# heathsc/bs_call

Hardware: AMD Instinct MI355X
Metric: genome positions called/sec (higher is better)
Workload: dtype f64; 1 GPU; configs[1]: synthetic chr22-sized contig, 50000000 positions at 30x WGBS (L-pileup generator), pile-ups resident in HBM, one contig per GPU; positions_per_gpu=50000000, coverage=30

## Files before the change

bs_call_amd/_lib.py:

```python
import ctypes as C
import os

HERE = os.path.dirname(os.path.abspath(__file__))
LIB_PATH = os.environ.get("BSCALL_AMD_LIB") or os.path.join(HERE, "lib", "libbscall_amd.so")

EXPORTS = (
    "bsc_abi_version",
    "bsc_last_error",
    "bsc_params_default",
    "bsc_create",
    "bsc_destroy",
    "bsc_get_tables",
    "bsc_phred_table",
    "bsc_call_sites",
    "bsc_alloc_host",
    "bsc_free_host",
    "bsc_call_sites_device",
    "bsc_accumulate",
    "bsc_accumulate_device",
    "bsc_block_status",
    "bsc_last_accumulate_ms",
    "bsc_call_block",
    "bsc_block_submit",
    "bsc_block_fetch",
    "bsc_block_submit_to",
    "bsc_synth_reads_host",
    "bsc_vcf_records",
# ... 412 lines not shown
    vp, u64, u32, i32 = C.c_void_p, C.c_uint64, C.c_uint32, C.c_int
    L.bsc_abi_version.restype = i32
    L.bsc_abi_version.argtypes = []
    if L.bsc_abi_version() != ABI_VERSION:
        raise ImportError("%s has ABI %d, this package mirrors ABI %d: rebuild with `make`" % (LIB_PATH, L.bsc_abi_version(), ABI_VERSION))
    L.bsc_last_error.restype = C.c_char_p
    L.bsc_last_error.argtypes = []
    L.bsc_params_default.restype = None
    L.bsc_params_default.argtypes = [C.POINTER(Params)]
    L.bsc_create.restype = i32
    L.bsc_create.argtypes = [C.POINTER(Params), C.POINTER(vp)]
    L.bsc_destroy.restype = i32
    L.bsc_destroy.argtypes = [vp]
    L.bsc_get_tables.restype = i32
    L.bsc_get_tables.argtypes = [vp, vp, vp]
    L.bsc_phred_table.restype = i32
    L.bsc_phred_table.argtypes = [vp, vp]
    L.bsc_call_sites.restype = i32
    L.bsc_call_sites.argtypes = [vp, vp, vp, u64, vp, u32, vp]
    L.bsc_alloc_host.restype = vp
    L.bsc_alloc_host.argtypes = [u64]
    L.bsc_free_host.restype = None
    L.bsc_free_host.argtypes = [vp]
    L.bsc_call_sites_device.restype = i32
    L.bsc_call_sites_device.argtypes = [vp, vp, vp, u64, vp, u32, vp, vp]
    L.bsc_accumulate.restype = i32
    L.bsc_accumulate.argtypes = [vp, vp, u32, vp, u64, u32, u32, vp]
    L.bsc_accumulate_device.restype = i32
    L.bsc_accumulate_device.argtypes = [vp, vp, u32, vp, u64, u32, u32, vp, vp]
    L.bsc_block_status.restype = i32
# ... 452 lines not shown
```

bs_call_amd/caller.py:

```python
import ctypes as C

import numpy as np

from . import _lib
from .abi import GT_METH, PILEUP, SITE_STATS, TEMPLATE, VCF_CORE, VCF_REC

SYNTH_NRUNS = 1


class BscError(RuntimeError):
    def __init__(self, code, msg):
        super().__init__("bscall_amd error %d: %s" % (code, msg))
        self.code = code


class BscInexactWarning(UserWarning):
    """Some pile-up sums left the range where the reference's float sums are exact (BSC_WARN_INEXACT)."""


def _check(rc):
    if rc == 1:
        import warnings

        warnings.warn(_lib.load().bsc_last_error().decode("utf-8", "replace"), BscInexactWarning, stacklevel=3)
# ... 252 lines not shown
        at = 0
        for k in pieces:
            z.write(data[at : at + k])
            at += k
            parts.append(z.take())
        if at < len(data):
            z.write(data[at:])
        parts.append(z.close())
        return b"".join(parts)

    def tables(self):
        q = np.zeros((44, 5), dtype=np.float64)
        lf = np.zeros(256, dtype=np.float64)
        _check(self._L.bsc_get_tables(self._h, _ptr(q), _ptr(lf)))
        return q, lf

    def call_sites(self, pile, ref, out_stride=200, out=None, skip=None):
        pile = np.ascontiguousarray(pile, dtype=PILEUP)
        ref = np.ascontiguousarray(ref, dtype=np.uint8)
        n = len(pile)
        if len(ref) != n:
            raise ValueError("pile and ref differ in length")
        if out is None:
            out = np.zeros(n, dtype=GT_METH) if out_stride == 200 else np.zeros((n, out_stride), dtype=np.uint8)
        if skip is None:
            skip = np.zeros(n, dtype=np.uint8)
        _check_dest("out", out, n * out_stride)
        _check_dest("skip", skip, n)
        _check(self._L.bsc_call_sites(self._h, _ptr(pile), _ptr(ref), n, _ptr(out), out_stride, _ptr(skip)))
        return out, skip
# ... 1104 lines not shown
```

bs_call_amd/csrc/bscall_api.c:

```c
#ifndef __HIP_PLATFORM_AMD__
#define __HIP_PLATFORM_AMD__ 1
#endif
#include <hip/hip_runtime_api.h>
#include <math.h>
#include <pthread.h>
#include <stdarg.h>
#include <stdio.h>
#include <stdlib.h>
#include <string.h>

#include "../../include/bscall_amd.h"
#include "devtables.h"
#include "bsmath.h"
#include "bsmath_tables.h"
#include "synth.h"
#include "dbsnpdev_core.h"
#include "tabix_int.h"

int bsc_dev_launch_call(const void *cts, const void *ref, uint64_t n, void *out, uint32_t out_dw, void *skip,
                        const void *tb, void *het_list, void *counters, int num_cus, void *stream, void *ev_start,
                        void *ev_mid, void *ev_stop);
int bsc_dev_launch_accumulate(const void *rd, const void *bin_off, const void *seq, uint32_t x, uint32_t y, uint32_t min_qual, void *cts,
                              void *counters, int num_cus, void *stream);
int bsc_dev_launch_bin_reads(const void *tpl, uint32_t nr, const void *seq, uint64_t seq_bytes, uint32_t x, uint32_t y, void *tflag,
                             void *bin_cnt, void *bin_off, void *bin_cur, void *scan_tmp, size_t scan_tmp_bytes, void *rd,
                             void *counters, void *stream);
uint32_t bsc_dev_n_bins(uint32_t n_sites);
int bsc_dev_launch_site_stats(const void *core, const void *gtm, uint32_t gtm_stride, const void *dbsnp, uint32_t n,
                              const void *tb, const void *logp, const void *carry_in, void *carry_out, void *stats,
                              void *pairs, int num_cus, void *stream);
int bsc_dev_launch_gc_cov_gtm(const void *core, const void *gtm, uint32_t gtm_stride, uint32_t n, const void *gc_bins, uint32_t n_bins,
                              uint32_t start_pos, void *table, int num_cus, void *stream);
int bsc_dev_launch_meth_eval(void *pairs, const void *tb, const void *logp, void *stats, const void *ovf_list,
                             const void *counters, int num_cus, void *stream);
int bsc_dev_scan_tmp_bytes(uint32_t n, size_t *bytes);
int bsc_dev_launch_stream_probe(const void *cts, const void *ref, uint64_t n, void *out, void *skip, int num_cus,
// ... 287 lines not shown
  size_t cap_fscr;
  hipEvent_t ev_rchain[2];
  int ev_rchain_valid;
  hipEvent_t ev_raw[2];
  int ev_raw_valid;
  int ref_resident;
  hipEvent_t ev_acc[2];
  int ev_acc_valid;
  hipStream_t s_in, s_out;
  hipEvent_t ev_in[2], ev_k[2], ev_out[2];
  void *p_cts[2], *p_ref[2], *p_out[2], *p_skip[2];
  size_t p_cap_cts[2], p_cap_ref[2], p_cap_out[2], p_cap_skip[2];
  int pipe_ready;
  int profiling;
#define BSC_EV_RING 32
  hipEvent_t ev[BSC_EV_RING][3];
  uint64_t ev_count;
};

static __thread char bsc_errbuf[512];

static int bsc_fail(int code, const char *fmt, ...) {
  va_list ap;
  va_start(ap, fmt);
  vsnprintf(bsc_errbuf, sizeof bsc_errbuf, fmt, ap);
  va_end(ap);
  return code;
}

typedef struct {
  int prev;
// ... 98 lines not shown
    ctx->q_prob[q][3] = t->ln_k_half[q] = log(0.5 + k);
    ctx->q_prob[q][4] = t->ln_k_one[q] = log(1.0 + k);
  }
  t->lfact[0] = t->lfact[1] = 0.0;
  double l = 0.0;
  for (int i = 2; i < 256; i++) {
    l += log((double)i);
    t->lfact[i] = l;
  }
  memcpy(t->log_tab, bsm_log_tab, sizeof t->log_tab);
  memcpy(t->exp_tab, bsm_exp_tab, sizeof t->exp_tab);
  t->under_conv = ctx->params.under_conv;
  t->over_conv = ctx->params.over_conv;
  t->lrb = log(ctx->params.ref_bias);
  t->lrb1 = log(0.5 * (1.0 + ctx->params.ref_bias));
}

int bsc_create(const bsc_params *params, bsc_context **out) {
  if (!out) return bsc_fail(BSC_ERR_ARG, "bsc_create: out is NULL");
  *out = NULL;
  bsc_params p;
  if (params) p = *params;
  else bsc_params_default(&p);
  if (!(p.under_conv >= 0.0 && p.under_conv < 1.0) || !(p.over_conv >= 0.0 && p.over_conv < 1.0) || !(p.ref_bias > 0.0))
    return bsc_fail(BSC_ERR_ARG, "bsc_create: conversion rates must be in [0,1) and ref_bias > 0");
  if (!((1.0 - p.under_conv) - p.over_conv >= 0x1p-20))
    return bsc_fail(BSC_ERR_ARG, "bsc_create: under_conv + over_conv must be < 1 (by at least 2^-20)");
  if (p.min_qual < 1) p.min_qual = 1;
  if (p.min_qual > 43) p.min_qual = 43;

// ... 235 lines not shown
  hipFree(ctx->d_raw);
  hipFree(ctx->d_rseq);
  hipFree(ctx->d_rms);
  hipFree(ctx->d_pprof);
  hipFree(ctx->d_pmax);
  hipFree(ctx->d_pused);
  hipFree(ctx->d_pmask);
  if (ctx->h_prep) hipHostFree(ctx->h_prep);
  hipFree(ctx->d_carry);
  hipFree(ctx->d_logp);
  hipFree(ctx->d_vout);
  hipFree(ctx->d_vdb);
  if (ctx->h_stage) hipHostFree(ctx->h_stage);
  if (ctx->h_cnt) hipHostFree(ctx->h_cnt);
  for (int r = 0; r < BSC_EV_RING; r++)
    for (int i = 0; i < 3; i++)
      if (ctx->ev[r][i]) hipEventDestroy(ctx->ev[r][i]);
  free(ctx);
  return BSC_OK;
}

int bsc_get_tables(const bsc_context *ctx, double *q_prob_44x5, double *lfact_256) {
  if (!ctx) return bsc_fail(BSC_ERR_ARG, "bsc_get_tables: ctx is NULL");
  if (q_prob_44x5) memcpy(q_prob_44x5, ctx->q_prob, sizeof ctx->q_prob);
  if (lfact_256) memcpy(lfact_256, ctx->host_tables.lfact, sizeof ctx->host_tables.lfact);
  return BSC_OK;
}

static int bsc_reserve(void **p, size_t *cap, size_t need) {
  if (need <= *cap) return BSC_OK;
  if (*p) {
    hipError_t e = hipFree(*p);
    *p = NULL;
// ... 37 lines not shown
int bsc_call_sites_device(bsc_context *ctx, const void *d_cts, const void *d_ref, uint64_t n, void *d_out,
                          uint32_t out_stride, void *d_skip, void *stream) {
  if (!ctx) return bsc_fail(BSC_ERR_ARG, "bsc_call_sites_device: ctx is NULL");
  int rc = bsc_check_stride(out_stride);
  if (rc) return rc;
  if (n == 0) return BSC_OK;
  if (!d_cts || !d_ref || !d_out || !d_skip) return bsc_fail(BSC_ERR_ARG, "bsc_call_sites_device: NULL buffer");
  if (((uintptr_t)d_cts & 15u) || ((uintptr_t)d_out & 15u))
    return bsc_fail(BSC_ERR_ARG, "bsc_call_sites_device: d_cts and d_out must be 16-byte aligned");
  BSC_ENTER(ctx);
  hipStream_t s = (hipStream_t)stream;
  uint64_t done = 0;
  while (done < n) {
    uint64_t m = n - done;
    if (m > ctx->max_launch) m = ctx->max_launch;
    rc = bsc_reserve(&ctx->d_het, &ctx->cap_het, (size_t)((m + 63u) / 64u) * 8u);
    if (rc) return rc;
    int e = bsc_dev_launch_call((const char *)d_cts + done * 104u, (const char *)d_ref + done, m,
                                (char *)d_out + done * out_stride, out_stride / 4u, (char *)d_skip + done,
                                ctx->d_tables, ctx->d_het, ctx->d_counters, ctx->num_cus, s,
                                ctx->profiling ? ctx->ev[ctx->ev_count % BSC_EV_RING][0] : NULL,
                                ctx->profiling ? ctx->ev[ctx->ev_count % BSC_EV_RING][1] : NULL,
                                ctx->profiling ? ctx->ev[ctx->ev_count % BSC_EV_RING][2] : NULL);
    if (ctx->profiling) ctx->ev_count++;
    if (e) return bsc_fail(BSC_ERR_HIP, "kernel launch failed: %s", hipGetErrorString((hipError_t)e));
    done += m;
  }
  ctx->sites += n;
  return BSC_OK;
}

#define BSC_PIPE_CHUNK (1u << 20)

static int bsc_pipe_init(bsc_context *ctx) {
  if (ctx->pipe_ready) return BSC_OK;
  HIP_TRY(hipStreamCreateWithFlags(&ctx->s_in, hipStreamNonBlocking));
  HIP_TRY(hipStreamCreateWithFlags(&ctx->s_out, hipStreamNonBlocking));
  for (int b = 0; b < 2; b++) {
// ... 553 lines not shown
  ctx->reads_fused = fused != 0;
  return BSC_OK;
}

int bsc_debug_fail_summary_alloc(bsc_context *ctx, int on) {
  if (!ctx) return bsc_fail(BSC_ERR_ARG, "bsc_debug_fail_summary_alloc: ctx is NULL");
  ctx->dbg_fail_summary = on != 0;
  return BSC_OK;
}

int bsc_set_profiling(bsc_context *ctx, int enable) {
  if (!ctx) return bsc_fail(BSC_ERR_ARG, "bsc_set_profiling: ctx is NULL");
  BSC_ENTER(ctx);
  if (enable && !ctx->ev[0][0])
    for (int r = 0; r < BSC_EV_RING; r++)
      for (int i = 0; i < 3; i++) HIP_TRY(hipEventCreate(&ctx->ev[r][i]));
  ctx->profiling = enable != 0;
  ctx->ev_count = 0;
  return BSC_OK;
}

int bsc_kernel_ms_history(bsc_context *ctx, uint32_t age, float *call_ms, float *fisher_ms) {
  if (!ctx) return bsc_fail(BSC_ERR_ARG, "bsc_kernel_ms_history: ctx is NULL");
  if (!ctx->profiling || age >= ctx->ev_count || age >= BSC_EV_RING)
    return bsc_fail(BSC_ERR_ARG, "bsc_kernel_ms_history: no profiled launch %u launches back (the last %d are kept)", age, BSC_EV_RING);
  BSC_ENTER(ctx);
  hipEvent_t *ev = ctx->ev[(ctx->ev_count - 1u - age) % BSC_EV_RING];
  HIP_TRY(hipEventSynchronize(ev[2]));
  float a = 0.f, b = 0.f;
  HIP_TRY(hipEventElapsedTime(&a, ev[0], ev[1]));
  HIP_TRY(hipEventElapsedTime(&b, ev[1], ev[2]));
  if (call_ms) *call_ms = a;
  if (fisher_ms) *fisher_ms = b;
  return BSC_OK;
}

int bsc_last_kernel_ms(bsc_context *ctx, float *call_ms, float *fisher_ms) { return bsc_kernel_ms_history(ctx, 0, call_ms, fisher_ms); }

int bsc_stream_probe_ms(bsc_context *ctx, const void *d_cts, const void *d_ref, uint64_t n, void *d_out, void *d_skip,
                        int reps, void *stream, float *ms) {
  if (!ctx || !d_cts || !d_ref || !d_out || !d_skip || !ms) return bsc_fail(BSC_ERR_ARG, "bsc_stream_probe_ms: NULL argument");
  if (((uintptr_t)d_cts & 15u) || ((uintptr_t)d_out & 15u))
    return bsc_fail(BSC_ERR_ARG, "bsc_stream_probe_ms: d_cts and d_out must be 16-byte aligned");
  BSC_ENTER(ctx);
  hipEvent_t a, b;
  HIP_TRY(hipEventCreate(&a));
  HIP_TRY(hipEventCreate(&b));
  float best = 0.f;
// ... 3738 lines not shown
```

bs_call_amd/csrc/bsmath.h:

```cpp
#ifndef BSCALL_AMD_BSMATH_H
#define BSCALL_AMD_BSMATH_H

#include <stdint.h>

#include "bsmath_tables.h"

#if defined(__HIPCC__)
#define BSM_FN __host__ __device__ static __forceinline__
#else
#define BSM_FN static inline __attribute__((always_inline))
#endif

#define BSM_FMA(a, b, c) __builtin_fma((a), (b), (c))

BSM_FN uint64_t bsm_bits(double x) {
  uint64_t u;
  __builtin_memcpy(&u, &x, 8);
  return u;
}
BSM_FN double bsm_from_bits(uint64_t u) {
  double x;
  __builtin_memcpy(&x, &u, 8);
  return x;
}
// ... 104 lines not shown
BSM_FN double bsm_lfact_big_t(int n, const double *logtab) {
  const double x = (double)(n + 1);
  const double t = bsm_log_t(x, logtab);
  const double z = 1.0 / x;
  const double y = z * z;
  double w = y * -1.63092934096575273989e-03;
  w = y * (8.36339918996282139126e-04 + w);
  w = y * (-5.95187557450339963135e-04 + w);
  w = y * (7.93650558643019558500e-04 + w);
  w = y * (-2.77777777728775536470e-03 + w);
  w = z * (8.33333333333329678849e-02 + w);
  w = 4.18938533204672725052e-01 + w;
  return (x - 0.5) * (t - 1.0) + w;
}

#if !defined(__HIPCC__)
BSM_FN double bsm_log(double x) { return bsm_log_t(x, bsm_log_tab); }
BSM_FN double bsm_exp(double x) { return bsm_exp_t(x, bsm_exp_tab); }
BSM_FN double bsm_lfact_big(int n) { return bsm_lfact_big_t(n, bsm_log_tab); }
#endif

#endif
```

bs_call_amd/csrc/callmath.h:

```cpp
#ifndef BSCALL_AMD_CALLMATH_H
#define BSCALL_AMD_CALLMATH_H

#include <hip/hip_runtime.h>
#include <stdint.h>

#include "bsmath.h"

#ifndef BSC_DMA_AUX
#define BSC_DMA_AUX 2
#endif
#define IN_DW 26
#define OUT_DW 50
#define MAX_OUT_DW 52
#define SLOT_DW (64 * IN_DW)

#define WAVE_LDS_ORDER()                                     \
  do {                                                       \
    __builtin_amdgcn_fence(__ATOMIC_RELEASE, "wavefront");   \
    __builtin_amdgcn_wave_barrier();                         \
    __builtin_amdgcn_fence(__ATOMIC_ACQUIRE, "wavefront");   \
  } while (0)

__device__ static __forceinline__ unsigned lane_rank(unsigned long long m) {
  return __builtin_amdgcn_mbcnt_hi((uint32_t)(m >> 32), __builtin_amdgcn_mbcnt_lo((uint32_t)m, 0u));
// ... 170 lines not shown
  const uint64_t db = bsm_bits(d);
  const bool allones = ((uint32_t)db & ((uint32_t)(db >> 32) | 0xfff00000u)) == 0xffffffffu;
  if (__builtin_expect(__any(allones), 0)) {
    s0 = allones ? n0 / d : s0;
    s1 = allones ? n1 / d : s1;
    s2 = allones ? n2 / d : s2;
  }
  s0 = s0 < -1.0 ? -1.0 : (s0 > 1.0 ? 1.0 : s0);
  Z0 = 0.5 * (lmt * s0 + 2.0 - lpt);
  s1 = s1 < -1.0 ? -1.0 : (s1 > 1.0 ? 1.0 : s1);
  Z1 = 0.5 * (lmt * s1 + 2.0 - lpt);
  s2 = s2 < -1.0 ? -1.0 : (s2 > 1.0 ? 1.0 : s2);
  Z2 = 0.5 * (lmt * s2 + 2.0 - lpt);
}

#define PT_Q 44
#define PT_A 0
#define PT_B 1
#define PT_C 2
#define PT_D 3
#define PT_E 4
#define PT_WORDS (5 * PT_Q)
__device__ static __forceinline__ double pure_log_entry(unsigned idx, double l, double t, const double *s_k, const double *logtab) {
  const unsigned id = idx / PT_Q, q = idx - id * PT_Q;
  const double lpt = l + t, lmt = l - t;
  const double Zc = 0.5 * (lmt * -1.0 + 2.0 - lpt), Zd = 0.5 * (lmt * 1.0 + 2.0 - lpt);
  const double k = s_k[q];
  double x;
  switch (id) {
    case PT_A: x = 1.0 - Zc + k; break;
    case PT_B: x = 1.0 - 0.5 * Zc + k; break;
    case PT_C: x = 0.5 * (1.0 - Zc) + k; break;
    case PT_D: x = Zd + k; break;
    default: x = 0.5 * Zd + k; break;
  }
  return bsm_log_t(x, logtab);
}

__device__ static __forceinline__ void dma16(const void *g, void *lds_wave_base) {
  __builtin_amdgcn_global_load_lds((const __attribute__((address_space(1))) void *)g,
                                   (__attribute__((address_space(3))) void *)lds_wave_base, 16, 0, BSC_DMA_AUX);
}

__device__ static __forceinline__ double lfact_dev(int x, const double *lf, const double *logtab) {
  return x < 256 ? lf[x] : bsm_lfact_big_t(x, logtab);
}

__device__ static double fisher_dev(int c0, int c1, int c2, int c3, const double *lf, const double *logtab,
                                    const uint64_t *exptab) {
#define LF(x) lfact_dev((x), lf, logtab)
  const int row0 = c0 + c1, row1 = c2 + c3, col0 = c0 + c2, col1 = c1 + c3;
  const int n = row0 + row1;
// ... 75 lines not shown
```

bs_call_amd/csrc/devtables.h:

```cpp
#ifndef BSCALL_AMD_DEVTABLES_H
#define BSCALL_AMD_DEVTABLES_H

#include <stdint.h>

typedef struct {
  double k[44], ln_k[44], ln_k_half[44], ln_k_one[44];
  double lfact[256];
  double log_tab[256];
  unsigned long long exp_tab[256];
  double under_conv, over_conv;
  double lrb, lrb1;
  double phred_thr[64][4];
  unsigned char phred_base[64];
} bsc_dev_tables;

#define BSC_CNT_HET_LIST 0
#define BSC_CNT_COVERED 1
#define BSC_CNT_SPAN 13
#define BSC_CNT_INEXACT 14
#define BSC_CNT_ERR 15
#define BSC_CNT_RECORDS 16
#define BSC_CNT_OVF 17
#define BSC_CNT_DEEP 18
#define BSC_CNT_WORDS 19

#define BSC_TERR_LEFT 1
#define BSC_TERR_ORI 2
#define BSC_TERR_STRAND 3
// ... 43 lines not shown
```

bs_call_amd/csrc/fused.hip:

```cpp
#include <hip/hip_runtime.h>
#include <stdint.h>
#include <stdlib.h>
#include <string.h>

#include "accdev.h"
#include "bsmath.h"
#include "callmath.h"
#include "devtables.h"
#include "sitestats_dev.h"

#ifndef FW
#define FW 16
#endif
#ifndef BSC_CHAIN_STAGGER
#define BSC_CHAIN_STAGGER 0
#endif
#define FT 60
#define FT2 62
#ifndef BSC_RUN_CAP
#define BSC_RUN_CAP 32
#endif
#define SUM_DW 12
#define F_COV_LDS 256
#define F_WORDS (SS_COV + F_COV_LDS * 6)
// ... 311 lines not shown
    s_lnk[tid] = tb->ln_k[tid];
    s_half[tid] = tb->ln_k_half[tid];
    s_one[tid] = tb->ln_k_one[tid];
  }
  if (tid < 256) {
    s_logtab[tid] = tb->log_tab[tid];
    s_exptab[tid] = tb->exp_tab[tid];
    s_pthr[tid] = (&tb->phred_thr[0][0])[tid];
  }
  if (tid < 64) s_pbase[tid] = tb->phred_base[tid];
  if (tid < 12) s_cnt[tid] = 0;
  if (a.with_stats) {
    for (unsigned i = tid; i < F_WORDS; i += 64 * FW) h[i] = 0;
    for (unsigned i = tid; i < 4 * F_PAIR * F_PAIR; i += 64 * FW) s_pair[i] = 0;
  }
  __syncthreads();
  if (tid < PT_WORDS) s_ptab[tid] = pure_log_entry(tid, K_COLD(l), K_COLD(t), s_k, s_logtab);
  if (tid >= 256 && tid < 306) {
    const unsigned r = (tid - 256u) / 10u, g = (tid - 256u) % 10u;
    int ga, gb;
    f_alleles((int)g, ga, gb);
    s_prior[tid - 256u] = r == 0 ? 0.0 : (ga == (int)r && gb == (int)r ? K_COLD(lrb) : ((ga == (int)r || gb == (int)r) ? K_COLD(lrb1) : 0.0));
  }
  __syncthreads();
  if (BSC_CHAIN_STAGGER)
    for (unsigned i = 0; i < wid; i++) __builtin_amdgcn_s_sleep(BSC_CHAIN_STAGGER);

  uint32_t *slot = lds_slot[wid];
  uint32_t *sg = s_gw[wid];
  uint16_t *srf = s_rf[wid];
  uint16_t *spd = s_pend[wid];
  int64_t ref_lo, ref_hi;
// ... 915 lines not shown
```

bs_call_amd/csrc/kernels.hip:

```cpp
#include <hip/hip_runtime.h>
#include <stdint.h>

#include "bsmath.h"
#include "callmath.h"
#include "devtables.h"
#include "synth.h"

#ifndef TILE
#define TILE 256
#endif
#ifndef BSC_TILES_PER_WAVE
#define BSC_TILES_PER_WAVE 16
#endif
#ifndef BSC_WAVES_PER_SIMD
#define BSC_WAVES_PER_SIMD 4
#endif

template <bool FULL>
__global__ __launch_bounds__(TILE, BSC_WAVES_PER_SIMD) void bsc_call_kernel_t(const uint32_t *__restrict__ cts,
                                                                      const uint8_t *__restrict__ ref,
                                                                      uint64_t n_sites, uint64_t wt_begin,
                                                                      uint64_t wt_end, uint32_t *__restrict__ out,
                                                                      uint32_t out_dw, uint8_t *__restrict__ skip,
                                                                      const bsc_dev_tables *__restrict__ tb,
                                                                      uint32_t *__restrict__ het_list,
                                                                      unsigned long long *__restrict__ counters) {
  __shared__ __attribute__((aligned(16))) uint32_t lds_slot[TILE / 64][SLOT_DW];
  __shared__ double s_k[44], s_lnk[44], s_half[44], s_one[44];
#ifdef BSC_TABLES_GLOBAL
  const double *const s_logtab = tb->log_tab;
  const unsigned long long *const s_exptab = tb->exp_tab;
#else
  __shared__ double s_logtab[256];
  __shared__ unsigned long long s_exptab[256];
#endif
  __shared__ unsigned int s_cnt[12];
  __shared__ double s_ptab[PT_WORDS];
  __shared__ uint8_t s_pairs[TILE / 64][256];

  const unsigned tid = threadIdx.x;
  const unsigned lane = tid & 63u;
  const unsigned wid = __builtin_amdgcn_readfirstlane(tid >> 6);
  if (tid < 44) {
    s_k[tid] = tb->k[tid];
    s_lnk[tid] = tb->ln_k[tid];
    s_half[tid] = tb->ln_k_half[tid];
    s_one[tid] = tb->ln_k_one[tid];
  }
#ifndef BSC_TABLES_GLOBAL
  for (unsigned i = tid; i < 256; i += TILE) {
    s_logtab[i] = tb->log_tab[i];
    s_exptab[i] = tb->exp_tab[i];
  }
#endif
  if (tid < 12) s_cnt[tid] = 0;
  const double l = 1.0 - tb->under_conv;
  const double t = tb->over_conv;
  const double lrb = tb->lrb, lrb1 = tb->lrb1;
  __syncthreads();
  for (unsigned i = tid; i < PT_WORDS; i += TILE) s_ptab[i] = pure_log_entry(i, l, t, s_k, s_logtab);
  __syncthreads();

  uint32_t *slot = lds_slot[wid];
  const uint32_t wave_stride = gridDim.x * (TILE / 64);
  const uint32_t wt_last = (uint32_t)wt_end;
  for (uint32_t wt = (uint32_t)wt_begin + blockIdx.x * (TILE / 64) + wid; wt < wt_last; wt += wave_stride) {
    const uint64_t site0 = (uint64_t)wt * 64;
    const unsigned nvalid = FULL ? 64u : (unsigned)((n_sites - site0) < 64 ? (n_sites - site0) : 64);
    const bool full = FULL;
    const uint64_t site = site0 + lane;
    const bool valid = FULL || lane < nvalid;
    const unsigned rf = valid ? ref[site] : 0u;

    uint32_t w[IN_DW];
    if (full) {
// ... 7 lines not shown
      for (int i = 0; i < IN_DW / 2; i++) {
        const uint2 v = rec[i];
        w[2 * i] = v.x;
        w[2 * i + 1] = v.y;
      }
    } else {
#pragma unroll
      for (int i = 0; i < IN_DW; i++) w[i] = valid ? cts[site * IN_DW + i] : 0u;
    }
#include "call_body.inc"
    const bool het = covered && ((0x16Eu >> mxi) & 1u);
    if (covered) {
      atomicAdd(&s_cnt[0], 1u);
      atomicAdd(&s_cnt[1 + mxi], 1u);
    }
    {
      const unsigned long long m = __ballot(het);
      if (lane == 0) {
        reinterpret_cast<unsigned long long *>(het_list)[wt] = m;
        if (m) atomicAdd(&s_cnt[11], (unsigned)__popcll(m));
      }
    }
    if (valid) skip[site] = covered ? 0 : 1;

#pragma unroll 1
    for (unsigned half = 0; half < 2; half++) {
      __builtin_amdgcn_wave_barrier();
      const bool mine = valid && (lane >> 5) == half;
      auto write_record = [&](auto *rec) {
        if (covered) {
#pragma unroll
          for (int j = 0; j < 8; j++) rec[j] = make_uint2(cnt[j], 0u);
          rec[8] = make_uint2(qpack0 & 0xffu, (qpack0 >> 8) & 0xffu);
          rec[9] = make_uint2((qpack0 >> 16) & 0xffu, qpack0 >> 24);
          rec[10] = make_uint2(qpack1 & 0xffu, (qpack1 >> 8) & 0xffu);
// ... 19 lines not shown
      if (full) {
        __builtin_amdgcn_wave_barrier();
        const unsigned nvec = 32u * out_dw / 4u;
        uint4 *dst = reinterpret_cast<uint4 *>(out + (site0 + half * 32u) * out_dw);
        const uint4 *srcv = reinterpret_cast<const uint4 *>(slot);
#pragma unroll
        for (unsigned v = 0; v < 7; v++) {
          const unsigned idx = v * 64u + lane;
          if (idx < nvec) {
            typedef unsigned int u32x4 __attribute__((ext_vector_type(4)));
            __builtin_nontemporal_store(reinterpret_cast<const u32x4 *>(srcv)[idx], reinterpret_cast<u32x4 *>(dst) + idx);
          }
        }
      }
    }
  }

  __syncthreads();
  if (tid < 12 && s_cnt[tid]) atomicAdd(&counters[BSC_CNT_COVERED + tid], (unsigned long long)s_cnt[tid]);
}

#define FI_THREADS 256
#define FI_LIST 2048
extern "C" __global__ __launch_bounds__(FI_THREADS) void bsc_fisher_kernel(const uint32_t *__restrict__ cts,
                                                                           uint32_t *__restrict__ out, uint32_t out_dw,
                                                                           const bsc_dev_tables *__restrict__ tb,
                                                                           const unsigned long long *__restrict__ masks,
                                                                           uint32_t n_tiles, uint32_t chunk_tiles) {
  __shared__ double s_lf[256];
  __shared__ double s_logtab[256];
  __shared__ unsigned long long s_exptab[256];
  __shared__ uint32_t s_scan[FI_THREADS + 1];
  __shared__ uint32_t s_list[FI_LIST];
  const unsigned tid = threadIdx.x;
  s_lf[tid] = tb->lfact[tid];
  s_logtab[tid] = tb->log_tab[tid];
  s_exptab[tid] = tb->exp_tab[tid];
  const uint32_t per = (chunk_tiles + FI_THREADS - 1) / FI_THREADS;
  for (uint32_t c0 = blockIdx.x * chunk_tiles; c0 < n_tiles; c0 += gridDim.x * chunk_tiles) {
    const uint32_t c1 = min(c0 + chunk_tiles, n_tiles);
    const uint32_t t0 = min(c0 + tid * per, c1), t1 = min(t0 + per, c1);
    uint32_t mine = 0;
    for (uint32_t t = t0; t < t1; t++) mine += (uint32_t)__popcll(masks[t]);
    __syncthreads();
    s_scan[tid + 1] = mine;
    if (tid == 0) s_scan[0] = 0;
    __syncthreads();
    if (tid < 64) {
      uint32_t a = s_scan[4 * tid + 1], b = a + s_scan[4 * tid + 2], c = b + s_scan[4 * tid + 3], d = c + s_scan[4 * tid + 4];
      uint32_t run = d;
#pragma unroll
      for (int off = 1; off < 64; off <<= 1) {
        const uint32_t v = __shfl_up(run, off);
        if ((int)tid >= off) run += v;
      }
      const uint32_t base = run - d;
      s_scan[4 * tid + 1] = base + a;
      s_scan[4 * tid + 2] = base + b;
      s_scan[4 * tid + 3] = base + c;
      s_scan[4 * tid + 4] = base + d;
    }
    __syncthreads();
    const uint32_t total = s_scan[FI_THREADS], first = s_scan[tid];
    for (uint32_t w0 = 0; w0 < total; w0 += FI_LIST) {
      if (w0) __syncthreads();
      if (first < w0 + FI_LIST && first + mine > w0) {
        uint32_t k = first;
        for (uint32_t t = t0; t < t1; t++) {
          unsigned long long m = masks[t];
          while (m) {
            const unsigned bit = (unsigned)__builtin_ctzll(m);
            m &= m - 1ull;
            if (k >= w0 && k < w0 + FI_LIST) s_list[k - w0] = t * 64u + bit;
            k++;
          }
        }
      }
      __syncthreads();
      const uint32_t cnt = min((uint32_t)FI_LIST, total - w0);
      for (uint32_t i = tid; i < cnt; i += FI_THREADS) {
        const uint64_t site = s_list[i];
        const uint32_t *p = cts + site * IN_DW;
        uint32_t f[8], r[8];
#pragma unroll
        for (int j = 0; j < 8; j++) {
          f[j] = p[j];
          r[j] = p[8 + j];
        }
        uint32_t *rec = out + site * out_dw;
        const unsigned mxi = rec[48] & 0xffu;
        int t0_, t1_, t2_, t3_;
        strand_table(mxi, f, r, t0_, t1_, t2_, t3_);
        double z = fisher_dev(t0_, t1_, t2_, t3_, s_lf, s_logtab, (const uint64_t *)s_exptab);
        if (z < 1.0e-20) z = 1.0e-20;
        const double fs = bsm_log_t(z, s_logtab) / BSM_LN10;
        const uint64_t b = bsm_bits(fs);
        reinterpret_cast<uint2 *>(rec)[22] = make_uint2((uint32_t)b, (uint32_t)(b >> 32));
      }
    }
  }
}

extern "C" __global__ __launch_bounds__(256) void bsc_synth_kernel(uint64_t seed, uint64_t first_site, uint64_t n,
                                                                   uint32_t coverage, uint32_t flags,
                                                                   uint32_t *__restrict__ cts,
                                                                   uint8_t *__restrict__ ref) {
  for (uint64_t i = (uint64_t)blockIdx.x * blockDim.x + threadIdx.x; i < n; i += (uint64_t)gridDim.x * blockDim.x) {
    uint32_t counts[16], nr, rf;
    float q[8], m2;
    syn_site(seed, first_site + i, coverage, flags, counts, &nr, q, &m2, &rf);
    uint32_t *p = cts + i * IN_DW;
#pragma unroll
    for (int j = 0; j < 16; j++) p[j] = counts[j];
    p[16] = nr;
#pragma unroll
    for (int j = 0; j < 8; j++) p[17 + j] = __float_as_uint(q[j]);
    p[25] = __float_as_uint(m2);
    ref[i] = (uint8_t)rf;
  }
}


extern "C" int bsc_dev_launch_call(const void *cts, const void *ref, uint64_t n, void *out, uint32_t out_dw, void *skip,
                                   const void *tb, void *het_list, void *counters, int num_cus, void *stream,
                                   void *ev_start, void *ev_mid, void *ev_stop) {
  if (n == 0) return 0;
  hipStream_t s = (hipStream_t)stream;
  if (ev_start) (void)hipEventRecord((hipEvent_t)ev_start, s);
  uint64_t resident = (uint64_t)num_cus * (BSC_WAVES_PER_SIMD * 4) / (TILE / 64);
  if (resident < 1) resident = 1;
  const uint64_t n_full = n / 64;
  hipError_t e = hipSuccess;
  if (n_full) {
    const uint64_t n_tiles = (n_full + (TILE / 64) - 1) / (TILE / 64);
    uint64_t rounds = n_full / (resident * (TILE / 64) * BSC_TILES_PER_WAVE);
    rounds = rounds < 1 ? 1 : (rounds > 16 ? 16 : rounds);
    uint64_t grid = resident * rounds;
    if (grid > n_tiles) grid = n_tiles;
    hipLaunchKernelGGL(bsc_call_kernel_t<true>, dim3((unsigned)grid), dim3(TILE), 0, s, (const uint32_t *)cts,
                       (const uint8_t *)ref, n, (uint64_t)0, n_full, (uint32_t *)out, out_dw, (uint8_t *)skip,
                       (const bsc_dev_tables *)tb, (uint32_t *)het_list, (unsigned long long *)counters);
    e = hipGetLastError();
    if (e != hipSuccess) return (int)e;
  }
  if (n & 63u) {
    hipLaunchKernelGGL(bsc_call_kernel_t<false>, dim3(1), dim3(TILE), 0, s, (const uint32_t *)cts, (const uint8_t *)ref, n,
                       n_full, n_full + 1, (uint32_t *)out, out_dw, (uint8_t *)skip, (const bsc_dev_tables *)tb,
                       (uint32_t *)het_list, (unsigned long long *)counters);
    e = hipGetLastError();
    if (e != hipSuccess) return (int)e;
  }
  if (ev_mid) (void)hipEventRecord((hipEvent_t)ev_mid, s);
  {
    const uint32_t n_tiles = (uint32_t)((n + 63) / 64);
    const uint32_t grid = (uint32_t)num_cus * 2u;
    uint32_t chunk = (n_tiles + grid - 1) / grid;
    chunk = chunk < 64u ? 64u : (chunk > 4096u ? 4096u : chunk);
    const uint32_t n_chunks = (n_tiles + chunk - 1) / chunk;
    hipLaunchKernelGGL(bsc_fisher_kernel, dim3(n_chunks < grid ? n_chunks : grid), dim3(FI_THREADS), 0, s, (const uint32_t *)cts,
                       (uint32_t *)out, out_dw, (const bsc_dev_tables *)tb, (const unsigned long long *)het_list, n_tiles, chunk);
  }
  e = hipGetLastError();
  if (ev_stop) (void)hipEventRecord((hipEvent_t)ev_stop, s);
  return (int)e;
}

extern "C" int bsc_dev_launch_synth(uint64_t seed, uint64_t first_site, uint64_t n, uint32_t coverage, uint32_t flags,
                                    void *cts, void *ref, int num_cus, void *stream) {
  if (n == 0) return 0;
  uint64_t grid = (n + 255) / 256;
  const uint64_t cap = (uint64_t)num_cus * 32u;
  if (grid > cap) grid = cap;
  hipLaunchKernelGGL(bsc_synth_kernel, dim3((unsigned)grid), dim3(256), 0, (hipStream_t)stream, seed, first_site, n,
                     coverage, flags, (uint32_t *)cts, (uint8_t *)ref);
  return (int)hipGetLastError();
}
```

include/bscall_amd.h:

```cpp
#ifndef BSCALL_AMD_H
#define BSCALL_AMD_H

#include <stddef.h>
#include <stdint.h>

#ifdef __cplusplus
extern "C" {
#endif

#define BSC_ABI_VERSION 2

#define BSC_OK 0
#define BSC_ERR_ARG (-1)
#define BSC_ERR_HIP (-2)
#define BSC_ERR_NOMEM (-3)
#define BSC_ERR_NO_DEVICE (-4)
#define BSC_ERR_RANGE (-5)
#define BSC_WARN_INEXACT 1

typedef struct {
  uint32_t counts[2][8];
  uint32_t n;
  float quality[8];
  float mapq2;
// ... 39 lines not shown
  uint64_t het_calls;
  uint64_t reserved[3];
} bsc_stats;

typedef struct bsc_context bsc_context;

int bsc_abi_version(void);
const char *bsc_last_error(void);
void bsc_params_default(bsc_params *p);

int bsc_create(const bsc_params *params, bsc_context **out);

int bsc_destroy(bsc_context *ctx);

int bsc_get_tables(const bsc_context *ctx, double *q_prob_44x5, double *lfact_256);

int bsc_phred_table(double *thr_64x4, unsigned char *base_64);

int bsc_call_sites(bsc_context *ctx, const bsc_pileup *cts, const uint8_t *ref, uint64_t n, void *out,
                   uint32_t out_stride, uint8_t *skip);

void *bsc_alloc_host(uint64_t bytes);
void bsc_free_host(void *p);

int bsc_call_sites_device(bsc_context *ctx, const void *d_cts, const void *d_ref, uint64_t n, void *d_out,
                          uint32_t out_stride, void *d_skip, void *stream);

int bsc_accumulate(bsc_context *ctx, const bsc_template *tpl, uint32_t nr, const uint8_t *seq, uint64_t seq_bytes,
                   uint32_t x, uint32_t y, bsc_pileup *out);

// ... 614 lines not shown
```

Before: 17.74 billion positions/s.

## Fuse Fisher strand test into call kernel and precompute pure-log table on host

Removes the separate Fisher kernel and the global het-site bitmask. Each call block now collects het sites in an LDS list and computes the Fisher strand p-values itself after the main loop. Long Fisher walks are spread across the wave with readlane, and sites that overflow the list are patched inline. The pure-log table is computed once on the host into the device tables instead of per block, which removes a syncthreads and the per-block logs. In exchange the call kernel uses more LDS and registers, which may lower occupancy, and the per-block Fisher tail is serialized after the main loop.

Result: no change. 17.67 billion positions/s (-0.4%).

```diff
diff --git a/bs_call_amd/_lib.py b/bs_call_amd/_lib.py
--- a/bs_call_amd/_lib.py
+++ b/bs_call_amd/_lib.py
@@ -11,6 +11,7 @@
     "bsc_create",
     "bsc_destroy",
     "bsc_get_tables",
+    "bsc_get_pure_logs",
     "bsc_phred_table",
     "bsc_call_sites",
     "bsc_alloc_host",
@@ -453,6 +454,8 @@
     L.bsc_destroy.argtypes = [vp]
     L.bsc_get_tables.restype = i32
     L.bsc_get_tables.argtypes = [vp, vp, vp]
+    L.bsc_get_pure_logs.restype = i32
+    L.bsc_get_pure_logs.argtypes = [vp, vp]
     L.bsc_phred_table.restype = i32
     L.bsc_phred_table.argtypes = [vp, vp]
     L.bsc_call_sites.restype = i32
diff --git a/bs_call_amd/caller.py b/bs_call_amd/caller.py
--- a/bs_call_amd/caller.py
+++ b/bs_call_amd/caller.py
@@ -290,6 +290,11 @@
         lf = np.zeros(256, dtype=np.float64)
         _check(self._L.bsc_get_tables(self._h, _ptr(q), _ptr(lf)))
         return q, lf
+
+    def pure_logs(self):
+        pt = np.zeros((5, 44), dtype=np.float64)
+        _check(self._L.bsc_get_pure_logs(self._h, _ptr(pt)))
+        return pt
 
     def call_sites(self, pile, ref, out_stride=200, out=None, skip=None):
         pile = np.ascontiguousarray(pile, dtype=PILEUP)
diff --git a/bs_call_amd/csrc/bscall_api.c b/bs_call_amd/csrc/bscall_api.c
--- a/bs_call_amd/csrc/bscall_api.c
+++ b/bs_call_amd/csrc/bscall_api.c
@@ -5,6 +5,7 @@
 #include <math.h>
 #include <pthread.h>
 #include <stdarg.h>
+#include <stddef.h>
 #include <stdio.h>
 #include <stdlib.h>
 #include <string.h>
@@ -18,8 +19,7 @@
 #include "tabix_int.h"
 
 int bsc_dev_launch_call(const void *cts, const void *ref, uint64_t n, void *out, uint32_t out_dw, void *skip,
-                        const void *tb, void *het_list, void *counters, int num_cus, void *stream, void *ev_start,
-                        void *ev_mid, void *ev_stop);
+                        const void *tb, void *counters, int num_cus, void *stream, void *ev_start, void *ev_stop);
 int bsc_dev_launch_accumulate(const void *rd, const void *bin_off, const void *seq, uint32_t x, uint32_t y, uint32_t min_qual, void *cts,
                               void *counters, int num_cus, void *stream);
 int bsc_dev_launch_bin_reads(const void *tpl, uint32_t nr, const void *seq, uint64_t seq_bytes, uint32_t x, uint32_t y, void *tflag,
@@ -337,7 +337,7 @@
   int pipe_ready;
   int profiling;
 #define BSC_EV_RING 32
-  hipEvent_t ev[BSC_EV_RING][3];
+  hipEvent_t ev[BSC_EV_RING][2];
   uint64_t ev_count;
 };
 
@@ -466,6 +466,8 @@
   t->over_conv = ctx->params.over_conv;
   t->lrb = log(ctx->params.ref_bias);
   t->lrb1 = log(0.5 * (1.0 + ctx->params.ref_bias));
+  const double pl = 1.0 - t->under_conv, pt = t->over_conv;
+  for (unsigned i = 0; i < PT_WORDS; i++) t->ptab[i] = pure_log_entry(i, pl, pt, t->k, t->log_tab);
 }
 
 int bsc_create(const bsc_params *params, bsc_context **out) {
@@ -731,9 +733,15 @@
   if (ctx->h_stage) hipHostFree(ctx->h_stage);
   if (ctx->h_cnt) hipHostFree(ctx->h_cnt);
   for (int r = 0; r < BSC_EV_RING; r++)
-    for (int i = 0; i < 3; i++)
+    for (int i = 0; i < 2; i++)
       if (ctx->ev[r][i]) hipEventDestroy(ctx->ev[r][i]);
   free(ctx);
+  return BSC_OK;
+}
+
+int bsc_get_pure_logs(const bsc_context *ctx, double *ptab_220) {
+  if (!ctx || !ptab_220) return bsc_fail(BSC_ERR_ARG, "bsc_get_pure_logs: NULL argument");
+  HIP_TRY(hipMemcpy(ptab_220, (const char *)ctx->d_tables + offsetof(bsc_dev_tables, ptab), sizeof ctx->host_tables.ptab, hipMemcpyDeviceToHost));
   return BSC_OK;
 }
 
@@ -801,14 +809,11 @@
   while (done < n) {
     uint64_t m = n - done;
     if (m > ctx->max_launch) m = ctx->max_launch;
-    rc = bsc_reserve(&ctx->d_het, &ctx->cap_het, (size_t)((m + 63u) / 64u) * 8u);
-    if (rc) return rc;
     int e = bsc_dev_launch_call((const char *)d_cts + done * 104u, (const char *)d_ref + done, m,
                                 (char *)d_out + done * out_stride, out_stride / 4u, (char *)d_skip + done,
-                                ctx->d_tables, ctx->d_het, ctx->d_counters, ctx->num_cus, s,
+                                ctx->d_tables, ctx->d_counters, ctx->num_cus, s,
                                 ctx->profiling ? ctx->ev[ctx->ev_count % BSC_EV_RING][0] : NULL,
-                                ctx->profiling ? ctx->ev[ctx->ev_count % BSC_EV_RING][1] : NULL,
-                                ctx->profiling ? ctx->ev[ctx->ev_count % BSC_EV_RING][2] : NULL);
+                                ctx->profiling ? ctx->ev[ctx->ev_count % BSC_EV_RING][1] : NULL);
     if (ctx->profiling) ctx->ev_count++;
     if (e) return bsc_fail(BSC_ERR_HIP, "kernel launch failed: %s", hipGetErrorString((hipError_t)e));
     done += m;
@@ -1392,7 +1397,7 @@
   BSC_ENTER(ctx);
   if (enable && !ctx->ev[0][0])
     for (int r = 0; r < BSC_EV_RING; r++)
-      for (int i = 0; i < 3; i++) HIP_TRY(hipEventCreate(&ctx->ev[r][i]));
+      for (int i = 0; i < 2; i++) HIP_TRY(hipEventCreate(&ctx->ev[r][i]));
   ctx->profiling = enable != 0;
   ctx->ev_count = 0;
   return BSC_OK;
@@ -1404,12 +1409,11 @@
     return bsc_fail(BSC_ERR_ARG, "bsc_kernel_ms_history: no profiled launch %u launches back (the last %d are kept)", age, BSC_EV_RING);
   BSC_ENTER(ctx);
   hipEvent_t *ev = ctx->ev[(ctx->ev_count - 1u - age) % BSC_EV_RING];
-  HIP_TRY(hipEventSynchronize(ev[2]));
-  float a = 0.f, b = 0.f;
+  HIP_TRY(hipEventSynchronize(ev[1]));
+  float a = 0.f;
   HIP_TRY(hipEventElapsedTime(&a, ev[0], ev[1]));
-  HIP_TRY(hipEventElapsedTime(&b, ev[1], ev[2]));
   if (call_ms) *call_ms = a;
-  if (fisher_ms) *fisher_ms = b;
+  if (fisher_ms) *fisher_ms = 0.f;
   return BSC_OK;
 }
 
diff --git a/bs_call_amd/csrc/bsmath.h b/bs_call_amd/csrc/bsmath.h
--- a/bs_call_amd/csrc/bsmath.h
+++ b/bs_call_amd/csrc/bsmath.h
@@ -142,6 +142,29 @@
   return (x - 0.5) * (t - 1.0) + w;
 }
 
+#define PT_Q 44
+#define PT_A 0
+#define PT_B 1
+#define PT_C 2
+#define PT_D 3
+#define PT_E 4
+#define PT_WORDS (5 * PT_Q)
+BSM_FN double pure_log_entry(unsigned idx, double l, double t, const double *s_k, const double *logtab) {
+  const unsigned id = idx / PT_Q, q = idx - id * PT_Q;
+  const double lpt = l + t, lmt = l - t;
+  const double Zc = 0.5 * (lmt * -1.0 + 2.0 - lpt), Zd = 0.5 * (lmt * 1.0 + 2.0 - lpt);
+  const double k = s_k[q];
+  double x;
+  switch (id) {
+    case PT_A: x = 1.0 - Zc + k; break;
+    case PT_B: x = 1.0 - 0.5 * Zc + k; break;
+    case PT_C: x = 0.5 * (1.0 - Zc) + k; break;
+    case PT_D: x = Zd + k; break;
+    default: x = 0.5 * Zd + k; break;
+  }
+  return bsm_log_t(x, logtab);
+}
+
 #if !defined(__HIPCC__)
 BSM_FN double bsm_log(double x) { return bsm_log_t(x, bsm_log_tab); }
 BSM_FN double bsm_exp(double x) { return bsm_exp_t(x, bsm_exp_tab); }
diff --git a/bs_call_amd/csrc/callmath.h b/bs_call_amd/csrc/callmath.h
--- a/bs_call_amd/csrc/callmath.h
+++ b/bs_call_amd/csrc/callmath.h
@@ -208,28 +208,6 @@
   Z2 = 0.5 * (lmt * s2 + 2.0 - lpt);
 }
 
-#define PT_Q 44
-#define PT_A 0
-#define PT_B 1
-#define PT_C 2
-#define PT_D 3
-#define PT_E 4
-#define PT_WORDS (5 * PT_Q)
-__device__ static __forceinline__ double pure_log_entry(unsigned idx, double l, double t, const double *s_k, const double *logtab) {
-  const unsigned id = idx / PT_Q, q = idx - id * PT_Q;
-  const double lpt = l + t, lmt = l - t;
-  const double Zc = 0.5 * (lmt * -1.0 + 2.0 - lpt), Zd = 0.5 * (lmt * 1.0 + 2.0 - lpt);
-  const double k = s_k[q];
-  double x;
-  switch (id) {
-    case PT_A: x = 1.0 - Zc + k; break;
-    case PT_B: x = 1.0 - 0.5 * Zc + k; break;
-    case PT_C: x = 0.5 * (1.0 - Zc) + k; break;
-    case PT_D: x = Zd + k; break;
-    default: x = 0.5 * Zd + k; break;
-  }
-  return bsm_log_t(x, logtab);
-}
 
 __device__ static __forceinline__ void dma16(const void *g, void *lds_wave_base) {
   __builtin_amdgcn_global_load_lds((const __attribute__((address_space(1))) void *)g,
diff --git a/bs_call_amd/csrc/devtables.h b/bs_call_amd/csrc/devtables.h
--- a/bs_call_amd/csrc/devtables.h
+++ b/bs_call_amd/csrc/devtables.h
@@ -2,6 +2,8 @@
 #define BSCALL_AMD_DEVTABLES_H
 
 #include <stdint.h>
+
+#include "bsmath.h"
 
 typedef struct {
   double k[44], ln_k[44], ln_k_half[44], ln_k_one[44];
@@ -12,6 +14,7 @@
   double lrb, lrb1;
   double phred_thr[64][4];
   unsigned char phred_base[64];
+  double ptab[PT_WORDS];
 } bsc_dev_tables;
 
 #define BSC_CNT_HET_LIST 0
diff --git a/bs_call_amd/csrc/fused.hip b/bs_call_amd/csrc/fused.hip
--- a/bs_call_amd/csrc/fused.hip
+++ b/bs_call_amd/csrc/fused.hip
@@ -349,8 +349,7 @@
     for (unsigned i = tid; i < F_WORDS; i += 64 * FW) h[i] = 0;
     for (unsigned i = tid; i < 4 * F_PAIR * F_PAIR; i += 64 * FW) s_pair[i] = 0;
   }
-  __syncthreads();
-  if (tid < PT_WORDS) s_ptab[tid] = pure_log_entry(tid, K_COLD(l), K_COLD(t), s_k, s_logtab);
+  if (tid < PT_WORDS) s_ptab[tid] = tb->ptab[tid];
   if (tid >= 256 && tid < 306) {
     const unsigned r = (tid - 256u) / 10u, g = (tid - 256u) % 10u;
     int ga, gb;
diff --git a/bs_call_amd/csrc/kernels.hip b/bs_call_amd/csrc/kernels.hip
--- a/bs_call_amd/csrc/kernels.hip
+++ b/bs_call_amd/csrc/kernels.hip
@@ -15,6 +15,116 @@
 #ifndef BSC_WAVES_PER_SIMD
 #define BSC_WAVES_PER_SIMD 4
 #endif
+#define HL_CAP 192
+
+#ifndef FI_COOP
+#define FI_COOP 16
+#endif
+__device__ static __forceinline__ void fisher_walk_lane(int a, int b, int c, int d, int cnt, double &l, double &p) {
+  for (int i = 0; i < cnt; i++) {
+    l *= (double)((a - i) * (b - i)) / (double)((c + i + 1) * (d + i + 1));
+    p += l;
+  }
+}
+__device__ static __forceinline__ double readlane_f64(double x, unsigned e) {
+  const uint64_t u = bsm_bits(x);
+  const uint32_t lo = (uint32_t)__builtin_amdgcn_readlane((int)(uint32_t)u, (int)e);
+  const uint32_t hi = (uint32_t)__builtin_amdgcn_readlane((int)(uint32_t)(u >> 32), (int)e);
+  return bsm_from_bits(((uint64_t)hi << 32) | lo);
+}
+__device__ static __forceinline__ void fisher_walk_wave(int a, int b, int c, int d, int cnt, double &l, double &p, unsigned lane) {
+  for (int base = 0; base < cnt; base += 64) {
+    const int i = base + (int)lane;
+    const double q = i < cnt ? (double)((a - i) * (b - i)) / (double)((c + i + 1) * (d + i + 1)) : 1.0;
+    const int m = cnt - base < 64 ? cnt - base : 64;
+    for (int j = 0; j < m; j++) {
+      l *= readlane_f64(q, (unsigned)j);
+      p += l;
+    }
+  }
+}
+__device__ static __forceinline__ void fisher_patch_wave(bool act, const uint32_t *__restrict__ cts, uint32_t *__restrict__ out,
+                                                         uint32_t out_dw, uint64_t site, unsigned mxi, const double *lf,
+                                                         const double *s_logtab, const unsigned long long *s_exptab, unsigned lane) {
+#define LF(x) lfact_dev((x), lf, s_logtab)
+  int aA = 0, bA = 0, cA = 0, dA = 0, nA = 0, aB = 0, bB = 0, cB = 0, dB = 0, nB = 0;
+  bool has2 = false;
+  double l0 = 1.0, l1 = 0.0;
+  if (act) {
+    const uint32_t *p = cts + site * IN_DW;
+    uint32_t f[8], r[8];
+#pragma unroll
+    for (int j = 0; j < 8; j++) {
+      f[j] = p[j];
+      r[j] = p[8 + j];
+    }
+    int c0, c1, c2, c3;
+    strand_table(mxi, f, r, c0, c1, c2, c3);
+    const int row0 = c0 + c1, row1 = c2 + c3, col0 = c0 + c2, col1 = c1 + c3;
+    const int n = row0 + row1;
+    if (n != 0) {
+      const double delta = (double)c0 - (double)(row0 * col0) / (double)n;
+      const double knst = LF(col0) + LF(col1) + LF(row0) + LF(row1) - LF(n);
+      l0 = bsm_exp_t(knst - LF(c0) - LF(c1) - LF(c2) - LF(c3), (const uint64_t *)s_exptab);
+      if (delta > 0.0) {
+        aA = c1; bA = c2; cA = c0; dA = c3;
+        nA = c1 < c2 ? c1 : c2;
+        const int mn = c0 < c3 ? c0 : c3;
+        const int k = (int)ceil(2.0 * delta);
+        if (k <= mn) {
+          c0 -= k; c3 -= k; c1 += k; c2 += k;
+          has2 = true;
+          aB = c0; bB = c3; cB = c1; dB = c2;
+          nB = mn - k;
+        }
+      } else {
+        aA = c0; bA = c3; cA = c1; dA = c2;
+        nA = c0 < c3 ? c0 : c3;
+        const int mn = c1 < c2 ? c1 : c2;
+        int k = (int)ceil(-2.0 * delta);
+        if (!k) k = 1;
+        if (k <= mn) {
+          c0 += k; c3 += k; c1 -= k; c2 -= k;
+          has2 = true;
+          aB = c1; bB = c2; cB = c0; dB = c3;
+          nB = mn - k;
+        }
+      }
+      if (has2) l1 = bsm_exp_t(knst - LF(c0) - LF(c1) - LF(c2) - LF(c3), (const uint64_t *)s_exptab);
+    }
+  }
+  double l = l0, z = l0;
+  const bool lng = act && nA + nB > FI_COOP;
+  if (act && !lng) {
+    fisher_walk_lane(aA, bA, cA, dA, nA, l, z);
+    if (has2) {
+      l = l1;
+      z += l;
+      fisher_walk_lane(aB, bB, cB, dB, nB, l, z);
+    }
+  }
+  const unsigned long long m2 = __ballot(has2);
+  for (unsigned long long ml = __ballot(lng); ml; ml &= ml - 1ull) {
+    const unsigned e = (unsigned)__builtin_ctzll(ml);
+#define RL(v) __builtin_amdgcn_readlane((v), (int)e)
+    double ul = readlane_f64(l0, e), uz = ul;
+    fisher_walk_wave(RL(aA), RL(bA), RL(cA), RL(dA), RL(nA), ul, uz, lane);
+    if ((m2 >> e) & 1ull) {
+      ul = readlane_f64(l1, e);
+      uz += ul;
+      fisher_walk_wave(RL(aB), RL(bB), RL(cB), RL(dB), RL(nB), ul, uz, lane);
+    }
+#undef RL
+    if (lane == e) z = uz;
+  }
+  if (act) {
+    if (z < 1.0e-20) z = 1.0e-20;
+    const double fs = bsm_log_t(z, s_logtab) / BSM_LN10;
+    const uint64_t b = bsm_bits(fs);
+    reinterpret_cast<uint2 *>(out + site * out_dw)[22] = make_uint2((uint32_t)b, (uint32_t)(b >> 32));
+  }
+#undef LF
+}
 
 template <bool FULL>
 __global__ __launch_bounds__(TILE, BSC_WAVES_PER_SIMD) void bsc_call_kernel_t(const uint32_t *__restrict__ cts,
@@ -23,7 +133,6 @@
                                                                       uint64_t wt_end, uint32_t *__restrict__ out,
                                                                       uint32_t out_dw, uint8_t *__restrict__ skip,
                                                                       const bsc_dev_tables *__restrict__ tb,
-                                                                      uint32_t *__restrict__ het_list,
                                                                       unsigned long long *__restrict__ counters) {
   __shared__ __attribute__((aligned(16))) uint32_t lds_slot[TILE / 64][SLOT_DW];
   __shared__ double s_k[44], s_lnk[44], s_half[44], s_one[44];
@@ -34,7 +143,11 @@
   __shared__ double s_logtab[256];
   __shared__ unsigned long long s_exptab[256];
 #endif
-  __shared__ unsigned int s_cnt[12];
+  __shared__ unsigned int s_cnt[11];
+  __shared__ unsigned int s_hn, s_hend;
+  __shared__ uint32_t s_hl[HL_CAP];
+  __shared__ uint8_t s_hg[HL_CAP];
+  __shared__ double s_lf[256];
   __shared__ double s_ptab[PT_WORDS];
   __shared__ uint8_t s_pairs[TILE / 64][256];
 
@@ -53,12 +166,13 @@
     s_exptab[i] = tb->exp_tab[i];
   }
 #endif
-  if (tid < 12) s_cnt[tid] = 0;
+  for (unsigned i = tid; i < 256; i += TILE) s_lf[i] = tb->lfact[i];
+  for (unsigned i = tid; i < PT_WORDS; i += TILE) s_ptab[i] = tb->ptab[i];
+  if (tid < 11) s_cnt[tid] = 0;
+  if (tid == 11) s_hn = s_hend = 0;
   const double l = 1.0 - tb->under_conv;
   const double t = tb->over_conv;
   const double lrb = tb->lrb, lrb1 = tb->lrb1;
-  __syncthreads();
-  for (unsigned i = tid; i < PT_WORDS; i += TILE) s_ptab[i] = pure_log_entry(i, l, t, s_k, s_logtab);
   __syncthreads();
 
   uint32_t *slot = lds_slot[wid];
@@ -96,11 +210,24 @@
       atomicAdd(&s_cnt[0], 1u);
       atomicAdd(&s_cnt[1 + mxi], 1u);
     }
+    bool self = false;
     {
       const unsigned long long m = __ballot(het);
-      if (lane == 0) {
-        reinterpret_cast<unsigned long long *>(het_list)[wt] = m;
-        if (m) atomicAdd(&s_cnt[11], (unsigned)__popcll(m));
+      if (m) {
+        const unsigned c = (unsigned)__popcll(m);
+        unsigned base = 0;
+        if (lane == 0) base = atomicAdd(&s_hn, c);
+        base = __builtin_amdgcn_readfirstlane(base);
+        if (base + c <= HL_CAP) {
+          if (het) {
+            const unsigned k = base + lane_rank(m);
+            s_hl[k] = (uint32_t)site;
+            s_hg[k] = (uint8_t)mxi;
+          }
+        } else {
+          if (base <= HL_CAP && lane == 0) s_hend = base;
+          self = true;
+        }
       }
     }
     if (valid) skip[site] = covered ? 0 : 1;
@@ -150,90 +277,24 @@
         }
       }
     }
-  }
-
+    if (__builtin_expect(self, 0)) {
+      asm volatile("s_waitcnt vmcnt(0)" ::: "memory");
+      fisher_patch_wave(het, cts, out, out_dw, site, (unsigned)mxi, s_lf, s_logtab, s_exptab, lane);
+    }
+  }
+
+  asm volatile("s_waitcnt vmcnt(0)" ::: "memory");
   __syncthreads();
-  if (tid < 12 && s_cnt[tid]) atomicAdd(&counters[BSC_CNT_COVERED + tid], (unsigned long long)s_cnt[tid]);
-}
-
-#define FI_THREADS 256
-#define FI_LIST 2048
-extern "C" __global__ __launch_bounds__(FI_THREADS) void bsc_fisher_kernel(const uint32_t *__restrict__ cts,
-                                                                           uint32_t *__restrict__ out, uint32_t out_dw,
-                                                                           const bsc_dev_tables *__restrict__ tb,
-                                                                           const unsigned long long *__restrict__ masks,
-                                                                           uint32_t n_tiles, uint32_t chunk_tiles) {
-  __shared__ double s_lf[256];
-  __shared__ double s_logtab[256];
-  __shared__ unsigned long long s_exptab[256];
-  __shared__ uint32_t s_scan[FI_THREADS + 1];
-  __shared__ uint32_t s_list[FI_LIST];
-  const unsigned tid = threadIdx.x;
-  s_lf[tid] = tb->lfact[tid];
-  s_logtab[tid] = tb->log_tab[tid];
-  s_exptab[tid] = tb->exp_tab[tid];
-  const uint32_t per = (chunk_tiles + FI_THREADS - 1) / FI_THREADS;
-  for (uint32_t c0 = blockIdx.x * chunk_tiles; c0 < n_tiles; c0 += gridDim.x * chunk_tiles) {
-    const uint32_t c1 = min(c0 + chunk_tiles, n_tiles);
-    const uint32_t t0 = min(c0 + tid * per, c1), t1 = min(t0 + per, c1);
-    uint32_t mine = 0;
-    for (uint32_t t = t0; t < t1; t++) mine += (uint32_t)__popcll(masks[t]);
-    __syncthreads();
-    s_scan[tid + 1] = mine;
-    if (tid == 0) s_scan[0] = 0;
-    __syncthreads();
-    if (tid < 64) {
-      uint32_t a = s_scan[4 * tid + 1], b = a + s_scan[4 * tid + 2], c = b + s_scan[4 * tid + 3], d = c + s_scan[4 * tid + 4];
-      uint32_t run = d;
-#pragma unroll
-      for (int off = 1; off < 64; off <<= 1) {
-        const uint32_t v = __shfl_up(run, off);
-        if ((int)tid >= off) run += v;
-      }
-      const uint32_t base = run - d;
-      s_scan[4 * tid + 1] = base + a;
-      s_scan[4 * tid + 2] = base + b;
-      s_scan[4 * tid + 3] = base + c;
-      s_scan[4 * tid + 4] = base + d;
-    }
-    __syncthreads();
-    const uint32_t total = s_scan[FI_THREADS], first = s_scan[tid];
-    for (uint32_t w0 = 0; w0 < total; w0 += FI_LIST) {
-      if (w0) __syncthreads();
-      if (first < w0 + FI_LIST && first + mine > w0) {
-        uint32_t k = first;
-        for (uint32_t t = t0; t < t1; t++) {
-          unsigned long long m = masks[t];
-          while (m) {
-            const unsigned bit = (unsigned)__builtin_ctzll(m);
-            m &= m - 1ull;
-            if (k >= w0 && k < w0 + FI_LIST) s_list[k - w0] = t * 64u + bit;
-            k++;
-          }
-        }
-      }
-      __syncthreads();
-      const uint32_t cnt = min((uint32_t)FI_LIST, total - w0);
-      for (uint32_t i = tid; i < cnt; i += FI_THREADS) {
-        const uint64_t site = s_list[i];
-        const uint32_t *p = cts + site * IN_DW;
-        uint32_t f[8], r[8];
-#pragma unroll
-        for (int j = 0; j < 8; j++) {
-          f[j] = p[j];
-          r[j] = p[8 + j];
-        }
-        uint32_t *rec = out + site * out_dw;
-        const unsigned mxi = rec[48] & 0xffu;
-        int t0_, t1_, t2_, t3_;
-        strand_table(mxi, f, r, t0_, t1_, t2_, t3_);
-        double z = fisher_dev(t0_, t1_, t2_, t3_, s_lf, s_logtab, (const uint64_t *)s_exptab);
-        if (z < 1.0e-20) z = 1.0e-20;
-        const double fs = bsm_log_t(z, s_logtab) / BSM_LN10;
-        const uint64_t b = bsm_bits(fs);
-        reinterpret_cast<uint2 *>(rec)[22] = make_uint2((uint32_t)b, (uint32_t)(b >> 32));
-      }
-    }
+  const unsigned n_het = s_hn;
+  const unsigned n_list = n_het <= HL_CAP ? n_het : s_hend;
+  for (unsigned i0 = 0; i0 + wid < n_list; i0 += TILE) {
+    const unsigned i = i0 + lane * (TILE / 64) + wid;
+    const bool act = i < n_list;
+    fisher_patch_wave(act, cts, out, out_dw, act ? s_hl[i] : 0u, act ? s_hg[i] : 0u, s_lf, s_logtab, s_exptab, lane);
+  }
+  if (tid < 12) {
+    const unsigned v = tid < 11 ? s_cnt[tid] : n_het;
+    if (v) atomicAdd(&counters[BSC_CNT_COVERED + tid], (unsigned long long)v);
   }
 }
 
@@ -258,8 +319,7 @@
 
 
 extern "C" int bsc_dev_launch_call(const void *cts, const void *ref, uint64_t n, void *out, uint32_t out_dw, void *skip,
-                                   const void *tb, void *het_list, void *counters, int num_cus, void *stream,
-                                   void *ev_start, void *ev_mid, void *ev_stop) {
+                                   const void *tb, void *counters, int num_cus, void *stream, void *ev_start, void *ev_stop) {
   if (n == 0) return 0;
   hipStream_t s = (hipStream_t)stream;
   if (ev_start) (void)hipEventRecord((hipEvent_t)ev_start, s);
@@ -275,28 +335,16 @@
     if (grid > n_tiles) grid = n_tiles;
     hipLaunchKernelGGL(bsc_call_kernel_t<true>, dim3((unsigned)grid), dim3(TILE), 0, s, (const uint32_t *)cts,
                        (const uint8_t *)ref, n, (uint64_t)0, n_full, (uint32_t *)out, out_dw, (uint8_t *)skip,
-                       (const bsc_dev_tables *)tb, (uint32_t *)het_list, (unsigned long long *)counters);
+                       (const bsc_dev_tables *)tb, (unsigned long long *)counters);
     e = hipGetLastError();
     if (e != hipSuccess) return (int)e;
   }
   if (n & 63u) {
     hipLaunchKernelGGL(bsc_call_kernel_t<false>, dim3(1), dim3(TILE), 0, s, (const uint32_t *)cts, (const uint8_t *)ref, n,
                        n_full, n_full + 1, (uint32_t *)out, out_dw, (uint8_t *)skip, (const bsc_dev_tables *)tb,
-                       (uint32_t *)het_list, (unsigned long long *)counters);
+                       (unsigned long long *)counters);
     e = hipGetLastError();
-    if (e != hipSuccess) return (int)e;
-  }
-  if (ev_mid) (void)hipEventRecord((hipEvent_t)ev_mid, s);
-  {
-    const uint32_t n_tiles = (uint32_t)((n + 63) / 64);
-    const uint32_t grid = (uint32_t)num_cus * 2u;
-    uint32_t chunk = (n_tiles + grid - 1) / grid;
-    chunk = chunk < 64u ? 64u : (chunk > 4096u ? 4096u : chunk);
-    const uint32_t n_chunks = (n_tiles + chunk - 1) / chunk;
-    hipLaunchKernelGGL(bsc_fisher_kernel, dim3(n_chunks < grid ? n_chunks : grid), dim3(FI_THREADS), 0, s, (const uint32_t *)cts,
-                       (uint32_t *)out, out_dw, (const bsc_dev_tables *)tb, (const unsigned long long *)het_list, n_tiles, chunk);
-  }
-  e = hipGetLastError();
+  }
   if (ev_stop) (void)hipEventRecord((hipEvent_t)ev_stop, s);
   return (int)e;
 }
diff --git a/include/bscall_amd.h b/include/bscall_amd.h
--- a/include/bscall_amd.h
+++ b/include/bscall_amd.h
@@ -77,6 +77,7 @@
 int bsc_destroy(bsc_context *ctx);
 
 int bsc_get_tables(const bsc_context *ctx, double *q_prob_44x5, double *lfact_256);
+int bsc_get_pure_logs(const bsc_context *ctx, double *ptab_220);
 
 int bsc_phred_table(double *thr_64x4, unsigned char *base_64);
 
```
